# cnosdb/cnosdb

Hardware: NVIDIA H100
Metric: decoded+aggregated points/s (higher is better)
Workload: dtype i64/f64

## Files before the change

cnosdb_b200/csrc/scan_kernels.cuh:

```cuda
#pragma once
#include <type_traits>

#include "cursors.cuh"

namespace tskv {

constexpr uint32_t FULL = 0xffffffffu;
constexpr int MAX_RANGES = 8;
constexpr int N_TK = 3;
constexpr int N_VK = 3;
constexpr int N_SERIAL_BINS = N_TK * N_VK;
constexpr uint32_t SHORT_PAGE_ROWS = 1024;
enum { BIN_SHORT_RLE_S8B = N_SERIAL_BINS, BIN_SHORT_S8B_S8B = N_SERIAL_BINS + 1, BIN_SHORT_RLE_GOR = N_SERIAL_BINS + 2,
       BIN_SHORT_S8B_GOR = N_SERIAL_BINS + 3 };
constexpr int N_BINS = N_SERIAL_BINS + 4;

enum { TK_RLE = 0, TK_S8B = 1, TK_GEN = 2 };
enum { VK_S8B = 0, VK_GOR = 1, VK_GEN = 2 };

__host__ __device__ inline int time_class(uint8_t dk) {
  return dk == DK_RLE_SC ? TK_RLE : dk == DK_S8B_SC ? TK_S8B : TK_GEN;
}
__host__ __device__ inline int value_class(uint8_t dk) {
  return dk == DK_S8B_ZZ ? VK_S8B : dk == DK_GORILLA ? VK_GOR : VK_GEN;
// ... 656 lines not shown
  if (P.width <= 0) {
    b.lo = INT64_MIN; b.hi = INT64_MAX; b.idx = 0; b.valid = true; b.floor_regime = false;
    return true;
  }
  const int64_t w = P.width;
  const int64_t cap = P.floor_cap;
  if (b.valid && b.floor_regime && t > b.hi && (uint64_t)t - (uint64_t)b.hi <= (uint64_t)w && t <= cap &&
      b.idx + 1 < P.n_buckets) {
    b.lo = b.hi + 1;
    b.hi = (int64_t)((uint64_t)b.hi + ((uint64_t)cap - (uint64_t)b.hi < (uint64_t)w ? (uint64_t)cap - (uint64_t)b.hi : (uint64_t)w));
    b.idx += 1;
    return true;
  }
  int64_t dividend = (int64_t)((uint64_t)t - (uint64_t)P.origin_mod + (uint64_t)w);
  int64_t rem = dividend % w;
  int64_t start = (int64_t)((uint64_t)t - (uint64_t)rem);
  int64_t diff = (int64_t)((uint64_t)start - (uint64_t)P.first_bucket_start);
  if (diff < 0 || diff % w != 0 || diff / w >= (int64_t)P.n_buckets) return false;
  b.idx = (uint32_t)(diff / w);
  const bool wrapped = t < P.wrap_lo;
  if (dividend >= 0) {
    const uint64_t room = (uint64_t)(wrapped ? P.wrap_lo - 1 : cap) - (uint64_t)start;
    b.lo = start;
    b.hi = (int64_t)((uint64_t)start + (room < (uint64_t)(w - 1) ? room : (uint64_t)(w - 1)));
  } else {
    b.lo = start - w + 1; b.hi = start;
    if (b.lo < P.wrap_lo) b.lo = P.wrap_lo;
  }
  b.floor_regime = dividend >= 0 && !wrapped;
  b.valid = true;
  return true;
}

__device__ __forceinline__ bool range_span(const ScanParams &P, int64_t t, int64_t &lo, int64_t &hi) {
  lo = INT64_MIN;
  hi = INT64_MAX;
  if (P.n_ranges == 0) return true;
  if (P.n_ranges == 1) {
    const int64_t a = P.ranges[0].min_ts, b = P.ranges[0].max_ts;
    if (t < a) { hi = a - 1; return false; }
    if (t > b) { lo = b + 1; return false; }
    lo = a; hi = b;
    return true;
  }
  bool in = false;
#pragma unroll 1
  for (uint32_t k = 0; k < P.n_ranges; k++) {
    const int64_t a = P.ranges[k].min_ts, b = P.ranges[k].max_ts;
    if (t >= a && t <= b) {
      if (!in) { lo = a; hi = b; in = true; }
    } else if (!in) {
      if (a > t && a - 1 < hi) hi = a - 1;
      if (b < t && a <= b && b + 1 > lo) lo = b + 1;
    }
  }
  return in;
}

__device__ __forceinline__ bool tomb_span(const tskv_time_range *r, uint32_t n, int64_t t, int64_t &lo, int64_t &hi) {
  bool in = false;
  int64_t l = INT64_MIN, h = INT64_MAX;
#pragma unroll 1
  for (uint32_t k = 0; k < n; k++) {
    const int64_t a = r[k].min_ts, b = r[k].max_ts;
    if (a > b) continue;
    if (t >= a && t <= b) {
      if (!in) { l = a; h = b; in = true; }
    } else if (!in) {
      if (a > t && a - 1 < h) h = a - 1;
      if (b < t && b + 1 > l) l = b + 1;
    }
  }
  lo = lo > l ? lo : l;
  hi = hi < h ? hi : h;
  return in;
}

__device__ __forceinline__ uint4 tomb_lookup(const ScanParams &P, uint32_t series, uint32_t column) {
  uint4 out = make_uint4(0, 0, 0, 0);
#pragma unroll 1
  for (int pass = 0; pass < 2; pass++) {
    const uint64_t key = ((uint64_t)series << 32) | (pass == 0 ? (uint64_t)TSKV_TOMB_ALL : (uint64_t)column);
    uint32_t lo = 0, hi = P.n_tomb_keys;
    while (lo < hi) {
      const uint32_t mid = (lo + hi) >> 1;
      if (__ldg(P.tomb_keys + mid) < key) lo = mid + 1;
      else hi = mid;
    }
    if (lo < P.n_tomb_keys && __ldg(P.tomb_keys + lo) == key) {
      const uint32_t a = __ldg(P.tomb_off + lo), b = __ldg(P.tomb_off + lo + 1);
      if (pass == 0) { out.x = a; out.y = b - a; }
      else { out.z = a; out.w = b - a; }
    }
  }
  return out;
}

template <int VK>
struct ValueAcc {
  uint32_t count;
  uint64_t sum;
  int64_t sum_hi;
  int64_t kmin, kmax;
  __device__ __forceinline__ void reset(bool narrow = false) {
    count = 0; sum = 0; sum_hi = 0;
    kmin = narrow ? INT32_MAX : INT64_MAX;
    kmax = narrow ? INT32_MIN : INT64_MIN;
  }
  __device__ __forceinline__ static int64_t with_lo(int64_t x, int32_t lo) {
    return (int64_t)(((uint64_t)x & 0xffffffff00000000ull) | (uint32_t)lo);
  }
  __device__ __forceinline__ void add32(uint32_t v) {
    sum += (uint64_t)(int64_t)(int32_t)v;
    kmin = with_lo(kmin, min((int32_t)kmin, (int32_t)v));
    kmax = with_lo(kmax, max((int32_t)kmax, (int32_t)v));
  }
  __device__ __forceinline__ void add(uint64_t v, uint8_t pt, uint64_t flip, bool  = false) {
    int64_t key;
    if (VK == VK_GOR || (VK == VK_GEN && pt == TSKV_PT_F64)) {
      sum = (uint64_t)__double_as_longlong(__longlong_as_double((long long)sum) + __longlong_as_double((long long)v));
      key = (int64_t)(v ^ (uint64_t)(((int64_t)v >> 63) & 0x7fffffffffffffffll));
    } else {
      sum += (uint32_t)v;
      sum_hi += pt == TSKV_PT_I64 ? (int64_t)(int32_t)(v >> 32) : (int64_t)(v >> 32);
      key = (int64_t)(v ^ flip);
    }
    kmin = key < kmin ? key : kmin;
    kmax = key > kmax ? key : kmax;
  }
  __device__ __forceinline__ void fold(uint8_t pt, bool narrow = false) {
    if (VK == VK_GOR || (VK == VK_GEN && pt == TSKV_PT_F64)) return;
    if (narrow) {
      const uint64_t flip = pt == TSKV_PT_U64 ? 0x8000000000000000ull : 0ull;
      sum_hi = (int64_t)sum >> 63;
      kmin = (int64_t)((uint64_t)(int64_t)(int32_t)kmin ^ flip);
      kmax = (int64_t)((uint64_t)(int64_t)(int32_t)kmax ^ flip);
      return;
    }
    const uint64_t x = (uint64_t)sum_hi << 32;
    const uint64_t lo = x + sum;
    sum_hi = (pt == TSKV_PT_I64 ? (sum_hi >> 32) : (int64_t)((uint64_t)sum_hi >> 32)) + (lo < x ? 1 : 0);
    sum = lo;
  }
};

#ifdef TSKV_FLUSH_SLOTS
constexpr int FLUSH_SLOTS = TSKV_FLUSH_SLOTS;
__host__ __device__ constexpr int flush_slots(int ) { return FLUSH_SLOTS; }
#else
constexpr int FLUSH_SLOTS = 4;
__host__ __device__ constexpr int flush_slots(int tk) { return tk == TK_S8B ? 2 : FLUSH_SLOTS; }
#endif
constexpr int FLUSH_Q = 5;
__host__ __device__ constexpr uint32_t flush_stage_bytes(int ns) { return (ns * FLUSH_Q * 32 + ns) * 8; }

template <int VK, int NS>
__device__ __forceinline__ void reduce_staged(const ScanParams &P, uint64_t *stab, uint64_t *stage, uint32_t n_slots) {
  __syncwarp();
  const uint32_t lane = threadIdx.x & 31;
  const uint32_t s = lane & (NS - 1), g = lane / NS;
  const uint64_t meta = stage[NS * FLUSH_Q * 32 + s];
  const uint32_t qcol = (uint32_t)(meta >> 32);
  const ColState &cs = P.cols[s < n_slots ? qcol : 0];
  const bool is_f64 = VK == VK_GOR || (VK == VK_GEN && cs.phys_type == TSKV_PT_F64);
  uint64_t cnt = 0, sum = 0;
  int64_t hi = 0, kmin = INT64_MAX, kmax = INT64_MIN;
  const uint64_t *base = stage + (size_t)s * FLUSH_Q * 32;
  static_assert(NS == 2 || NS == 4, "reduce_staged: lane j owns slot j % NS");
#pragma unroll
  for (int i = 0; i < NS; i++) {
    const uint32_t src = g * NS + ((i + s) & (NS - 1));
    const uint64_t c = base[src], v = base[32 + src];
    cnt += c;
    if (is_f64) {
      sum = (uint64_t)__double_as_longlong(__longlong_as_double((long long)sum) + __longlong_as_double((long long)v));
    } else {
      sum += v;
      if (VK != VK_GOR) hi += (int64_t)base[64 + src] + (sum < v ? 1 : 0);
    }
    const int64_t a = (int64_t)base[96 + src], b = (int64_t)base[128 + src];
    kmin = a < kmin ? a : kmin;
    kmax = b > kmax ? b : kmax;
  }
#pragma unroll
  for (int o = NS; o < 32; o <<= 1) {
    cnt += shfl_xor_u64(cnt, o);
    const uint64_t v = shfl_xor_u64(sum, o);
    const int64_t vh = VK != VK_GOR ? (int64_t)shfl_xor_u64((uint64_t)hi, o) : 0;
    if (is_f64) {
      sum = (uint64_t)__double_as_longlong(__longlong_as_double((long long)sum) + __longlong_as_double((long long)v));
    } else {
      sum += v;
      if (VK != VK_GOR) hi += vh + (sum < v ? 1 : 0);
    }
    const int64_t a = (int64_t)shfl_xor_u64((uint64_t)kmin, o), b = (int64_t)shfl_xor_u64((uint64_t)kmax, o);
    kmin = a < kmin ? a : kmin;
    kmax = b > kmax ? b : kmax;
  }
  if (lane < n_slots && cnt)
    table_update(P, stab, cs, (uint64_t)(uint32_t)meta, cs.agg_mask, is_f64, (uint32_t)cnt, sum, hi, kmin, kmax);
  __syncwarp();
}

template <int VK, int NS>
__device__ __forceinline__ void stage_partial(const ScanParams &P, uint64_t *stab, uint64_t *stage, uint32_t &seq, bool live,
                                              const ValueAcc<VK> &va, bool meta_lane, uint64_t gcell) {
  uint64_t *q = stage + (size_t)seq * FLUSH_Q * 32 + (threadIdx.x & 31);
  q[0] = live ? va.count : 0;
  q[32] = live ? va.sum : 0;
  if (VK != VK_GOR) q[64] = live ? (uint64_t)va.sum_hi : 0;
  q[96] = live ? (uint64_t)va.kmin : (uint64_t)INT64_MAX;
  q[128] = live ? (uint64_t)va.kmax : (uint64_t)INT64_MIN;
  if (meta_lane) stage[NS * FLUSH_Q * 32 + seq] = gcell;
  if (++seq == NS) {
    reduce_staged<VK, NS>(P, stab, stage, seq);
    seq = 0;
  }
}

template <int VK, int NS>
__device__ __forceinline__ void flush_runs(const ScanParams &P, uint64_t *stab, uint64_t *stage, uint32_t &seq, bool active,
                                           uint32_t qcol, uint64_t cell, uint8_t pt, uint8_t mask, const ValueAcc<VK> &va) {
  const uint32_t m = __ballot_sync(FULL, active);
  if (m == 0) return;
  const uint32_t lane = threadIdx.x & 31;
  const uint64_t gcell = ((uint64_t)qcol << 32) | (uint32_t)cell;
  const int leader = __ffs(m) - 1;
  const uint64_t lcell = shfl_u64(gcell, leader);
  const bool same = !P.group_by_series && __all_sync(FULL, !active || gcell == lcell);
  if (same) {
    stage_partial<VK, NS>(P, stab, stage, seq, active && va.count, va, (int)lane == leader, lcell);
  } else if (active && va.count) {
    table_update(P, stab, P.cols[qcol], cell, mask, VK == VK_GOR || (VK == VK_GEN && pt == TSKV_PT_F64), va.count, va.sum,
                 va.sum_hi, va.kmin, va.kmax);
  }
}

template <int K, typename S>
__device__ __forceinline__ bool cursor_exhausted(const DeltaCursor<K, S> &c) { return c.exhausted; }
template <bool ZZ>
__device__ __forceinline__ bool cursor_exhausted(const S8bCursor<ZZ> &c) { return c.exhausted(); }
template <int K, typename S>
__device__ __forceinline__ void cursor_reset(DeltaCursor<K, S> &c, uint32_t lane_ring) { c.bs.reset(lane_ring); }
template <bool ZZ>
__device__ __forceinline__ void cursor_reset(S8bCursor<ZZ> &c, uint32_t lane_ring) { c.reset(lane_ring); }

__device__ __forceinline__ uint32_t rle_rows_within(uint64_t d, uint64_t delta, double inv, uint32_t left) {
  const double e = (double)d * inv;
  if (e >= (double)left) return left;
  uint64_t q = (uint64_t)e;
  if (__umul64hi(q, delta) != 0 || q * delta > d) q--;
  else if (d - q * delta >= delta) q++;
  return (uint32_t)min((uint64_t)left, q + 1);
}

__device__ __forceinline__ uint32_t edge_rows(const ScanParams &P, uint32_t b, uint64_t t, uint64_t delta, double inv) {
  if (b >= P.n_buckets) return 1u;
  const int64_t end = __ldg(P.edges + b + 1);
  return (int64_t)t < end ? rle_rows_within((uint64_t)end - 1 - t, delta, inv, 0xffffffffu) : 0u;
}

struct GenTimeCursor : DeltaCursor<-1, BeStream> {
  const uint32_t *bm = nullptr;
  uint32_t word = 0;
  bool none = false;
};

template <int TK, int VK, bool SEL, bool NARROW, bool EDGES>
__device__ __forceinline__ void scan_chunk_seg(const ScanParams &P, uint32_t item_begin, uint32_t item_end,
                                               uint32_t ring_base, uint64_t *stab, uint64_t *stage, uint4 *s_tomb,
                                               uint32_t part, uint32_t n_parts, uint32_t part_rows) {
  constexpr int NS = flush_slots(TK);
  const uint32_t lane = threadIdx.x & 31;
  const uint32_t item = item_begin + lane;
  const bool have_item = item < item_end;
  const uint32_t tslot = ring_base + lane * RING_BYTES;
  const uint32_t vslot = ring_base + (TK == TK_S8B ? RING_BYTES_PER_WARP : 0) + lane * RING_BYTES;

  uint32_t page = 0, slot = 0, qcol = 0, n_rows = 0;
  uint8_t pt = VK == VK_GOR ? TSKV_PT_F64 : TSKV_PT_I64, mask = 0;
  PageView tpv, vpv;
  typename std::conditional<TK == TK_GEN, GenTimeCursor, S8bCursor<false>>::type tcur;
  uint64_t rle_t0 = 0, rle_delta = 0;
  double rle_inv = 0.0;
  typename std::conditional<VK == VK_S8B, S8bCursor<true>, DeltaCursor<-1, SeqStream>>::type vcur_d;
  GorillaRing vcur_g;
  const uint32_t *vbm = nullptr;
  const uint32_t *keepw = nullptr;
  bool allnull = false;
  int64_t pend_t = 0;

  if constexpr (TK == TK_S8B) tcur.reset(tslot);
  if (VK == VK_GOR) vcur_g.reset(vslot);
  else cursor_reset(vcur_d, vslot);
  uint32_t r0 = 0, page_rows = 0;
  if (have_item) {
    page = P.work_page[item];
    slot = P.work_slot[item];
    qcol = P.work_qcol[item] & 0x7f;
    const tskv_page_desc vd = P.descs[page];
    if (P.has_tomb) s_tomb[threadIdx.x] = tomb_lookup(P, vd.series_id, vd.column_id);
    const uint32_t tpage = P.time_page_of[page];
    const tskv_page_desc td = P.descs[tpage];
    if (VK != VK_GOR) pt = P.cols[qcol].phys_type;
    mask = P.cols[qcol].agg_mask;
    page_rows = vd.num_values;
    uint32_t sk_v = SKIP_NONE, sk_t = SKIP_NONE;
    bool split = false;
    if (n_parts > 1 && page_rows > part_rows) {
      sk_v = __ldg(P.skip_off + page);
      sk_t = TK == TK_S8B ? __ldg(P.skip_off + tpage) : 0u;
      split = sk_v != SKIP_NONE && sk_t != SKIP_NONE;
    }
    r0 = part * part_rows;
    tskv_status st = kind_status(vd.reserved);
    uint32_t st_page = page;
    if constexpr (TK == TK_GEN) {
      if (kind_status(td.reserved) != TSKV_OK) { st = kind_status(td.reserved); st_page = tpage; }
    }
    if (part != 0 && (!split || r0 >= page_rows)) {
    } else if (st != TSKV_OK) {
      report_error(P, st, st_page);
    } else {
      tpv.open(P.arena, td);
      vpv.open(P.arena, vd);
      n_rows = split ? min(page_rows, r0 + part_rows) : page_rows;
      vbm = reinterpret_cast<const uint32_t *>(vpv.bitset);
      if (P.row_keep) keepw = P.row_keep + P.keep_off[tpage];
      const uint32_t ent = r0 / SKIP_ROWS - 1;
      if (TK == TK_RLE) {
        DeltaCursor<DK_RLE_SC, BeStream> rc;
        st = rc.open(tpv, td.reserved);
        rle_delta = rc.delta;
        rle_t0 = rc.v + rc.delta;
        if ((int64_t)rle_delta > 0) rle_inv = 1.0 / (double)rle_delta;
      } else if (part == 0) {
        st = tcur.open(tpv, td.reserved, tslot);
      } else if constexpr (TK == TK_S8B) {
        tcur.restore(tpv, tslot, load_skip(P.skip + sk_t + ent));
      }
      if (st == TSKV_OK) {
        if (part == 0) {
          if (VK == VK_GOR) vcur_g.open(vpv, vslot);
          else { st = vcur_d.open(vpv, vd.reserved, vslot); allnull = vd.reserved == DK_ALLNULL; }
        } else {
          const SkipEntry e = load_skip(P.skip + sk_v + ent);
          if constexpr (VK == VK_GOR) vcur_g.restore(vpv, vslot, e);
          else if constexpr (VK == VK_S8B) vcur_d.restore(vpv, vslot, e);
        }
      }
      if constexpr (TK == TK_GEN) {
        if (td.reserved == DK_ALLNULL) n_rows = 0;
        tcur.bm = reinterpret_cast<const uint32_t *>(tpv.bitset);
      }
      if (st == TSKV_OK && n_rows) {
        if (TK == TK_RLE) {
          pend_t = (int64_t)(rle_t0 + (uint64_t)r0 * rle_delta);
        } else if constexpr (TK == TK_GEN) {
          uint32_t f = 0, w = 0;
          while (f < n_rows && (w = __ldg(tcur.bm + (f >> 5))) == 0) f += 32;
          if (f < n_rows) f += __ffs(w) - 1;
          tcur.none = f >= n_rows;
          if (f == 0) {
            pend_t = (int64_t)tcur.next();
          } else if (!tcur.none) {
            tcur.skip_first_if_s8b_sc();
            DeltaCursor<-1, BeStream> peek = tcur;
            pend_t = (int64_t)peek.next();
          }
          tcur.word = __ldg(tcur.bm);
        } else if (part == 0) {
          pend_t = (int64_t)tcur.next();
        } else {
          pend_t = (int64_t)tcur.v;
        }
      }
      if (st != TSKV_OK) { report_error(P, st, st == TSKV_ERR_BITSET_MISMATCH ? tpage : page); n_rows = 0; }
    }
  }
  const bool to_page_end = n_rows == page_rows;
  ring_drain();

  static_assert(!NARROW || (VK == VK_S8B && !SEL), "narrow chunks: simple8b integer values, no FIRST / LAST");
  ValueAcc<VK> va;
  va.reset(NARROW);
  RunAcc acc;
  acc.first_ts = acc.last_ts = 0; acc.first_val = acc.last_val = 0; acc.first_ok = acc.last_ok = false;
  BucketState bk; bk.valid = false; bk.floor_regime = false; bk.lo = 0; bk.hi = 0; bk.idx = 0;
  bool have_run = false;
  uint32_t run_idx = 0;
  uint32_t row = r0;
  if (n_rows == 0) row = 0;
  uint32_t n_points = 0, n_inrange = 0;
  uint32_t vword = 0, vahead = vbm ? __ldg(vbm + (row >> 5)) : 0;
  uint32_t kword = 0xffffffffu;
  bool first_pending = false;
  const uint64_t flip = pt == TSKV_PT_U64 ? 0x8000000000000000ull : 0ull;
  const uint64_t group_base = SEL ? 0 : group_cell_base<EDGES>(P, slot);
  uint32_t staged = 0;

  auto flush_now = [&](bool flush) {
    if (flush) va.fold(pt, NARROW);
    if (SEL) {
      if (__any_sync(FULL, flush)) {
        acc.count = va.count; acc.sum = va.sum; acc.sum_hi = va.sum_hi; acc.kmin = va.kmin; acc.kmax = va.kmax;
        const uint32_t fslot = have_item ? __ldg(P.work_slot + item) : 0u;
        warp_flush<SEL, EDGES>(P, stab, flush, qcol, group_cell_base<EDGES>(P, fslot) + bucket_cell<EDGES>(P, run_idx, flush),
                               (int64_t)run_idx, pt, mask, acc, fslot);
      }
    } else {
      flush_runs<VK, NS>(P, stab, stage, staged, flush, qcol, group_base + bucket_cell<EDGES>(P, run_idx, flush), pt, mask, va);
    }
  };
  auto row_value = [&](bool accumulate, bool &vv, bool &kept) -> uint64_t {
    if ((row & 31) == 0) {
      vword = vahead;
      vahead = __ldg(vbm + (row >> 5) + 1);
      if constexpr (TK == TK_GEN) kword = (keepw ? __ldg(keepw + (row >> 5)) : 0xffffffffu) & tcur.word;
      else if (keepw) kword = __ldg(keepw + (row >> 5));
    }
    vv = ((vword >> (row & 31)) & 1) && !allnull;
    kept = (kword >> (row & 31)) & 1;
    uint64_t v = 0;
    if (vv) {
      n_points++;
      if constexpr (NARROW) {
        const uint32_t v32 = vcur_d.next32();
        if (accumulate && kept) { va.count++; va.add32(v32); }
      } else {
        v = VK == VK_GOR ? vcur_g.next() : vcur_d.next();
        if (accumulate && kept) { va.count++; va.add(v, pt, flip); }
      }
    }
    return v;
  };
  auto next_add = [&](bool take) {
    if constexpr (NARROW) {
      const uint32_t v32 = vcur_d.next32();
      if (take) va.add32(v32);
    } else {
      const uint64_t v = VK == VK_GOR ? vcur_g.next() : vcur_d.next();
      if (take) va.add(v, pt, flip);
    }
  };
  auto check_values = [&]() {
    const bool bad = VK == VK_GOR ? vcur_g.failed() : cursor_exhausted(vcur_d);
    if (bad) {
      report_error(P, (VK == VK_GOR && vcur_g.overran()) ? TSKV_ERR_SHORT_BLOCK : TSKV_ERR_BITSET_MISMATCH, page);
      n_rows = 0;
      have_run = false;
    }
  };

  uint32_t ra = 0, rb1 = 0, nb = 0xffffffffu, q32 = 0, bidx = 0;
  uint64_t e_off = 0, w_rem = 0;
  bool fast = false;
  if (TK == TK_RLE) {
    bool elig = P.n_ranges <= 1 && !P.has_tomb;
    if (elig && n_rows) {
      const uint64_t span_t = (uint64_t)(page_rows - 1) * rle_delta;
      elig = (int64_t)rle_delta > 0 && __umul64hi((uint64_t)(page_rows - 1), rle_delta) == 0 && span_t < (1ull << 62) &&
             rle_t0 + (1ull << 62) < (1ull << 63) && rle_t0 + span_t + (1ull << 62) < (1ull << 63) &&
             P.width < ((int64_t)1 << 61);
      if (elig) {
        const int64_t t0 = (int64_t)rle_t0;
        ra = 0;
        rb1 = page_rows;
        if (P.n_ranges == 1) {
          const int64_t a = P.ranges[0].min_ts, b = P.ranges[0].max_ts;
          ra = a <= t0 ? 0u : rle_rows_within((uint64_t)(a - 1) - rle_t0, rle_delta, rle_inv, page_rows);
          rb1 = b < t0 ? 0u : rle_rows_within((uint64_t)b - rle_t0, rle_delta, rle_inv, page_rows);
        }
        ra = min(max(ra, row), n_rows);
        rb1 = min(max(rb1, row), n_rows);
        if ((P.width > 0 || EDGES) && ra < rb1) {
          const int64_t tr = (int64_t)(rle_t0 + (uint64_t)ra * rle_delta);
          if (P.width > 0 && (int64_t)((uint64_t)tr - (uint64_t)P.origin_mod + (uint64_t)P.width) < 0) {
            elig = false;
          } else if (!locate_bucket<EDGES>(P, tr, bk)) {
            report_error(P, TSKV_ERR_BUCKET_RANGE, page);
            n_rows = 0;
          } else {
            bidx = bk.idx;
            nb = rle_rows_within((uint64_t)bk.hi - (uint64_t)tr, rle_delta, rle_inv, 0xffffffffu);
            if (P.width > 0) {
              e_off = (uint64_t)tr + (uint64_t)nb * rle_delta - ((uint64_t)bk.hi + 1);
              q32 = rle_rows_within((uint64_t)P.width, rle_delta, rle_inv, 0xffffffffu) - 1;
              w_rem = (uint64_t)P.width - (uint64_t)q32 * rle_delta;
            }
          }
        }
      }
    }
    fast = __all_sync(FULL, elig);
  }

  if (TK == TK_RLE && VK != VK_GEN && !SEL && fast && (P.width > 0 || EDGES) && !P.group_by_series) {
    const bool mine = row < n_rows;
    const uint32_t with_rows = __ballot_sync(FULL, mine);
    const int src = with_rows ? __ffs(with_rows) - 1 : 0;
    const uint64_t t_first = rle_t0 + (uint64_t)row * rle_delta;
    const bool agree = (shfl_u64(rle_delta, src) == rle_delta) & (shfl_u64(t_first, src) == t_first) &
                       (shfl_u64(e_off, src) == e_off) & (__shfl_sync(FULL, row, src) == row) &
                       (__shfl_sync(FULL, n_rows, src) == n_rows) & (__shfl_sync(FULL, ra, src) == ra) &
                       (__shfl_sync(FULL, rb1, src) == rb1) & (__shfl_sync(FULL, bidx, src) == bidx) &
                       (__shfl_sync(FULL, nb, src) == nb) & (__shfl_sync(FULL, qcol, src) == qcol) &
                       (__shfl_sync(FULL, (uint32_t)group_base, src) == (uint32_t)group_base);
    if (with_rows && __all_sync(FULL, !mine || agree)) {
      rle_delta = shfl_u64(rle_delta, src);
      e_off = shfl_u64(e_off, src);
      w_rem = shfl_u64(w_rem, src);
      q32 = __shfl_sync(FULL, q32, src);
      row = __shfl_sync(FULL, row, src);
      ra = __shfl_sync(FULL, ra, src);
      rb1 = __shfl_sync(FULL, rb1, src);
      bidx = __shfl_sync(FULL, bidx, src);
      nb = __shfl_sync(FULL, nb, src);
      if (EDGES) {
        rle_t0 = shfl_u64(rle_t0, src);
        rle_inv = __longlong_as_double((long long)shfl_u64((uint64_t)__double_as_longlong(rle_inv), src));
      }
      const uint64_t col = ((uint64_t)__shfl_sync(FULL, qcol, src) << 32) | __shfl_sync(FULL, (uint32_t)group_base, src);
      uint32_t end = __shfl_sync(FULL, n_rows, src);
      while (row < end) {
        if (n_rows) {
          vword = vahead;
          vahead = __ldg(vbm + (row >> 5) + 1);
          if (keepw) kword = __ldg(keepw + (row >> 5));
        }
        const uint32_t wend = min(row + 32, end);
        const uint32_t m = (n_rows && !allnull) ? vword & (0xffffffffu >> (32 - (wend - row))) : 0u;
        const uint32_t lo = min(max(ra, row), wend) - row, hi = max(min(max(rb1, row), wend) - row, lo);
        const uint32_t take = m & kword & (uint32_t)((1ull << hi) - (1ull << lo));
        const bool dense = __all_sync(FULL, take == m);
        uint32_t r = row;
        while (r < wend) {
          const bool in = r >= ra && r < rb1;
          uint32_t pend = r < ra ? min(ra, wend) : wend;
          if (in) {
            if (nb == 0) {
              if (EDGES) {
                do {
                  bidx++;
                  nb = edge_rows(P, bidx, rle_t0 + (uint64_t)r * rle_delta, rle_delta, rle_inv);
                } while (nb == 0);
              } else {
                do {
                  bidx++;
                  nb = q32 + (e_off < w_rem ? 1u : 0u);
                  e_off = e_off + (uint64_t)nb * rle_delta - (uint64_t)P.width;
                } while (nb == 0);
              }
// ... 58 lines not shown
            } else {
              nb = q32 + (e_off < w_rem ? 1u : 0u);
              e_off = e_off + (uint64_t)nb * rle_delta - (uint64_t)P.width;
            }
          }
          if (bidx >= P.n_buckets) {
            report_error(P, TSKV_ERR_BUCKET_RANGE, page);
            seg_in = false;
            n_rows = row;
            pending = false;
          } else {
            seg_n = min(nb, rb1 - row);
            seg_b = bidx;
            if (P.width > 0 || EDGES) nb -= seg_n;
          }
        }
      } else {
        lim_lo = lim_hi = pend_t;
        seg_in = range_span(P, pend_t, lim_lo, lim_hi);
        if constexpr (TK == TK_GEN) seg_in = seg_in && !tcur.none;
        if (P.has_tomb) {
          const uint4 tl = s_tomb[threadIdx.x];
          const bool dropped = tomb_span(P.tomb_ranges, P.n_tomb_global, pend_t, lim_lo, lim_hi) |
                               tomb_span(P.tomb_ranges + tl.x, tl.y, pend_t, lim_lo, lim_hi);
          seg_masked = tomb_span(P.tomb_ranges + tl.z, tl.w, pend_t, lim_lo, lim_hi);
          if (dropped) seg_in = false;
        }
        if (seg_in) {
          if (!(bk.valid && pend_t >= bk.lo && pend_t <= bk.hi) && !locate_bucket<EDGES>(P, pend_t, bk)) {
            report_error(P, TSKV_ERR_BUCKET_RANGE, page);
            seg_in = false;
            bk.valid = false;
            lim_lo = lim_hi = pend_t;
          } else {
            lim_lo = lim_lo > bk.lo ? lim_lo : bk.lo;
            lim_hi = lim_hi < bk.hi ? lim_hi : bk.hi;
            seg_b = bk.idx;
          }
        }
        if (TK == TK_RLE) {
          const uint32_t left = n_rows - row;
          if ((int64_t)rle_delta > 0) {
            seg_n = rle_rows_within((uint64_t)lim_hi - (uint64_t)pend_t, rle_delta, rle_inv, left);
          } else {
            int64_t t = pend_t;
            do {
              seg_n++;
              t = (int64_t)((uint64_t)t + rle_delta);
            } while (seg_n < left && t >= lim_lo && t <= lim_hi);
          }
        }
      }
    }
    bool go = pending;
    if (align) {
      const uint32_t bmin = __reduce_min_sync(FULL, (pending && seg_in) ? seg_b : 0xffffffffu);
      go = pending && (!seg_in || seg_b == bmin);
    }
    const bool newrun = go && seg_in && (!have_run || seg_b != run_idx);
    const bool flush = have_run && (newrun || !has);
    flush_now(flush);
    if (flush) have_run = false;
    if (newrun) {
      have_run = true;
      run_idx = seg_b;
      va.reset(NARROW);
      if (SEL) { acc.first_ok = acc.last_ok = false; first_pending = true; }
    }
    if (go) {
      pending = false;
      const bool accumulate = seg_in && !seg_masked;
      if (TK == TK_RLE) {
        const uint32_t rend = row + seg_n;
        uint32_t r = row;
        while (r < rend) {
          if ((r & 31) == 0) {
            vword = vahead;
            vahead = __ldg(vbm + (r >> 5) + 1);
            if (keepw) kword = __ldg(keepw + (r >> 5));
          }
          const uint32_t off = r & 31;
          const uint32_t span = min(32u - off, rend - r);
          const uint32_t smask = 0xffffffffu >> (32 - span);
          const uint32_t m = allnull ? 0u : ((vword >> off) & smask);
          const uint32_t kb = (kword >> off) & smask;
          n_points += __popc(m);
          if (seg_in) n_inrange += __popc(kb);
          if (!SEL) {
            const uint32_t take = accumulate ? (m & kb) : 0u;
            va.count += __popc(take);
            if (__all_sync(__activemask(), take == m)) {
#pragma unroll 1
              for (uint32_t n = __popc(m); n; n--) next_add(true);
            } else {
#pragma unroll 1
              for (uint32_t b = m; b; b &= b - 1) next_add(take & b & (0u - b));
            }
          } else {
            for (uint32_t j = 0; j < span; j++) {
              bool vv = (m >> j) & 1;
              uint64_t v = 0;
              if (vv) v = VK == VK_GOR ? vcur_g.next() : vcur_d.next();
              vv = vv && !seg_masked;
              if (seg_in && ((kb >> j) & 1)) {
                const int64_t t = (int64_t)(rle_t0 + (uint64_t)(r + j) * rle_delta);
                if (first_pending) { acc.first_ts = t; acc.first_val = vv ? v : 0; acc.first_ok = vv; first_pending = false; }
                acc.last_ts = t;
                acc.last_val = vv ? v : 0;
                acc.last_ok = vv;
                if (vv) { va.count++; va.add(v, pt, flip); }
              }
            }
          }
          r += span;
        }
        row = rend;
        if (!(TK == TK_RLE && fast)) pend_t = (int64_t)(rle_t0 + (uint64_t)rend * rle_delta);
      } else {
        int64_t t = pend_t;
        const uint64_t span = (uint64_t)lim_hi - (uint64_t)lim_lo;
        bool more;
#pragma unroll 1
        do {
          bool vv, kept;
          const uint64_t v = row_value(accumulate, vv, kept);
          if (SEL && seg_in && kept) {
            const bool ok = vv && !seg_masked;
            if (first_pending) { acc.first_ts = t; acc.first_val = ok ? v : 0; acc.first_ok = ok; first_pending = false; }
            acc.last_ts = t;
            acc.last_val = ok ? v : 0;
            acc.last_ok = ok;
          }
          if (seg_in && kept) n_inrange++;
          row++;
          if constexpr (TK == TK_GEN) {
            if (row < n_rows) {
              if ((row & 31) == 0) tcur.word = __ldg(tcur.bm + (row >> 5));
              if ((tcur.word >> (row & 31)) & 1) t = (int64_t)tcur.next();
            }
          } else {
            t = (int64_t)tcur.next();
          }
          more = row < n_rows && (uint64_t)t - (uint64_t)lim_lo <= span;
        } while (more);
        pend_t = t;
        if (cursor_exhausted(tcur) && (TK == TK_GEN || row < n_rows)) {
          report_error(P, TSKV_ERR_BITSET_MISMATCH, P.time_page_of[page]);
          n_rows = row;
        }
      }
      check_values();
    }
  }
  if (!SEL && staged) {
    reduce_staged<VK, NS>(P, stab, stage, staged);
    staged = 0;
  }
  if (VK == VK_GOR && have_item && n_rows != 0 && to_page_end && vcur_g.consumed_any() && !vcur_g.drain())
    report_error(P, TSKV_ERR_SHORT_BLOCK, page);
  ring_drain();
  n_points = __reduce_add_sync(FULL, n_points);
  n_inrange = __reduce_add_sync(FULL, n_inrange);
  if (lane == 0) {
    if (n_points) atomicAdd(&P.stats[0], (unsigned long long)n_points);
    if (n_inrange) atomicAdd(&P.stats[1], (unsigned long long)n_inrange);
  }
}

#ifndef SCAN_MIN_BLOCKS
#define SCAN_MIN_BLOCKS 4
#endif
__host__ __device__ constexpr int scan_min_blocks(int , bool ) { return SCAN_MIN_BLOCKS; }
__host__ __device__ constexpr uint32_t scan_ring_bytes_per_warp(int tk) {
  return tk == TK_S8B ? 2 * RING_BYTES_PER_WARP : RING_BYTES_PER_WARP;
}
__host__ __device__ constexpr uint32_t scan_warp_bytes(int tk) {
  return scan_ring_bytes_per_warp(tk) + flush_stage_bytes(flush_slots(tk));
}
constexpr uint32_t SCAN_TOMB_BYTES = SCAN_THREADS * sizeof(uint4);
enum { NARROW_NONE = 0, NARROW_SOME = 1, NARROW_ALL = 2 };
template <int TK, int VK, bool SEL, int NARROW, bool EDGES>
__global__ void __launch_bounds__(SCAN_THREADS, scan_min_blocks(TK, SEL)) k_scan_aggregate(const __grid_constant__ ScanParams P, int bin) {
  static_assert(NARROW == NARROW_NONE || (TK != TK_GEN && VK == VK_S8B && !SEL), "narrow kernels: simple8b values, no FIRST / LAST");
  extern __shared__ __align__(16) uint64_t s_tab[];
  if (P.use_smem) {
    for (uint32_t i = threadIdx.x; i < P.smem_words; i += SCAN_THREADS) s_tab[i] = 0;
    __syncthreads();
    for (uint32_t c = 0; c < P.n_cols; c++) {
      const ColState cs = P.cols[c];
      for (uint32_t i = threadIdx.x; i < (uint32_t)P.n_cells; i += SCAN_THREADS) {
        if (cs.agg_mask & TSKV_AGG_MIN) s_tab[cs.s_min + i] = 0x7fffffffffffffffull;
        if (cs.agg_mask & TSKV_AGG_MAX) s_tab[cs.s_max + i] = 0x8000000000000000ull;
      }
    }
    __syncthreads();
  }
  const uint32_t lane = threadIdx.x & 31;
  uint64_t *warp_area = s_tab + ((P.smem_words + 1) & ~1u) + (size_t)(threadIdx.x >> 5) * (scan_warp_bytes(TK) / 8);
  const uint32_t ring_base = (uint32_t)__cvta_generic_to_shared(warp_area);
  uint64_t *stage = warp_area + scan_ring_bytes_per_warp(TK) / 8;
  uint4 *s_tomb = reinterpret_cast<uint4 *>(s_tab + ((P.smem_words + 1) & ~1u) + (SCAN_THREADS / 32) * (scan_warp_bytes(TK) / 8));
  uint32_t n_groups = 0;
  for (uint32_t k = bin * P.n_cols * WL_SUB; k < (bin + 1) * P.n_cols * WL_SUB; k++) n_groups += (__ldg(P.region_fill + k) + 31) >> 5;
  const uint32_t n_parts = (TK == TK_GEN || VK == VK_GEN || SEL) ? 1u : P.bin_parts[bin];
  const uint32_t part_rows = P.bin_part_rows[bin];
  const uint32_t n_chunks = n_groups * n_parts;
  for (;;) {
    uint32_t c = 0;
    if (lane == 0) c = atomicAdd(P.task_counter + bin, 1u);
    c = __shfl_sync(FULL, c, 0);
    if (c >= n_chunks) break;
    uint32_t group = n_parts > 1 ? c / n_parts : c;
    const uint32_t part = c - group * n_parts;
    uint32_t k = bin * P.n_cols * WL_SUB;
    asm("" : "+r"(k));
    uint32_t fill = __ldg(P.region_fill + k);
    while (group >= (fill + 31) >> 5) {
      group -= (fill + 31) >> 5;
      fill = __ldg(P.region_fill + ++k);
    }
    const uint32_t region = __ldg(P.region_start + k);
    const uint32_t begin = region + (group << 5);
    const uint32_t end = min(begin + 32, region + fill);
    if constexpr (NARROW == NARROW_SOME) {
      const uint32_t item = begin + lane;
      const bool narrow = __all_sync(FULL, item >= end || __ldg(P.page_narrow + __ldg(P.work_page + item)));
      if (narrow) scan_chunk_seg<TK, VK, SEL, true, EDGES>(P, begin, end, ring_base, s_tab, stage, s_tomb, part, n_parts, part_rows);
      else scan_chunk_seg<TK, VK, SEL, false, EDGES>(P, begin, end, ring_base, s_tab, stage, s_tomb, part, n_parts, part_rows);
    } else {
      scan_chunk_seg<TK, VK, SEL, NARROW == NARROW_ALL, EDGES>(P, begin, end, ring_base, s_tab, stage, s_tomb, part, n_parts, part_rows);
    }
  }
  if (P.use_smem) {
    __syncthreads();
    for (uint32_t c = 0; c < P.n_cols; c++) {
      const ColState cs = P.cols[c];
      const bool f64 = cs.phys_type == TSKV_PT_F64;
      for (uint32_t i = threadIdx.x; i < (uint32_t)P.n_cells; i += SCAN_THREADS) {
        const uint64_t cnt = s_tab[cs.s_count + i];
        if (!cnt) continue;
        atomicAdd(reinterpret_cast<unsigned long long *>(P.state + cs.count_off + i), (unsigned long long)cnt);
        if (cs.agg_mask & (TSKV_AGG_SUM | TSKV_AGG_MEAN)) {
          const uint64_t sv = s_tab[cs.s_sum + i];
          if (f64) atomicAdd(reinterpret_cast<double *>(P.state + cs.sum_off + i), __longlong_as_double((long long)sv));
          else add_int_sum(P.state + cs.sum_off + i, P.state + cs.sumhi_off + i, cs.agg_mask, sv,
                           (cs.agg_mask & TSKV_AGG_MEAN) ? (int64_t)s_tab[cs.s_hi + i] : 0);
        }
        if (cs.agg_mask & TSKV_AGG_MIN) atomicMin(reinterpret_cast<long long *>(P.state + cs.min_off + i), (long long)s_tab[cs.s_min + i]);
        if (cs.agg_mask & TSKV_AGG_MAX) atomicMax(reinterpret_cast<long long *>(P.state + cs.max_off + i), (long long)s_tab[cs.s_max + i]);
      }
    }
  }
}

struct StateLayout {
  uint64_t sum_i64_off, sum_i64_len;
  uint64_t sum_f64_off, sum_f64_len;
  uint64_t min_off, min_len;
  uint64_t max_off, max_len;
  uint64_t selval_off, selval_len;
  uint64_t first_pairs_off, first_cells;
  uint64_t last_pairs_off, last_cells;
  uint64_t first_keys_off, last_keys_off;
  uint64_t snap_off;
  uint64_t total;
};

constexpr uint32_t AUX_TASK_COUNTERS = 0;
constexpr uint32_t AUX_STATUS = 8;
constexpr uint32_t AUX_ERR_PAGE = 9;
constexpr uint32_t AUX_STATS = 10;
constexpr uint32_t AUX_COUNTERS = 12;
constexpr uint32_t AUX_CRC_STATUS = AUX_COUNTERS + N_COUNTERS;
constexpr uint32_t AUX_CRC_ERR_PAGE = AUX_CRC_STATUS + 1;
constexpr uint32_t AUX_WORDS = 32;
static_assert(N_BINS * 4 <= (AUX_STATUS - AUX_TASK_COUNTERS) * 8 && AUX_CRC_ERR_PAGE < AUX_WORDS, "scan aux block layout");

__global__ void k_init_state(uint64_t *state, StateLayout L, unsigned long long *aux, uint32_t aux_words, uint32_t *zero32,
                             uint32_t n_zero32) {
  uint64_t i = (uint64_t)blockIdx.x * blockDim.x + threadIdx.x;
  uint64_t stride = (uint64_t)gridDim.x * blockDim.x;
  for (uint64_t k = i; k < aux_words; k += stride) aux[k] = 0;
  for (uint64_t k = i; k < n_zero32; k += stride) zero32[k] = 0;
  for (uint64_t k = i; k < L.total; k += stride) {
    uint64_t v = 0;
    if (k >= L.min_off && k < L.min_off + L.min_len) v = 0x7fffffffffffffffull;
    else if (k >= L.max_off && k < L.max_off + L.max_len) v = 0x8000000000000000ull;
    else if (k >= L.first_pairs_off && k < L.first_pairs_off + 2 * L.first_cells) v = ((k - L.first_pairs_off) & 1) ? 0 : 0x7fffffffffffffffull;
    else if (k >= L.last_pairs_off && k < L.last_pairs_off + 2 * L.last_cells) v = ((k - L.last_pairs_off) & 1) ? 0 : 0x8000000000000000ull;
    state[k] = v;
  }
}

struct MeanExport {
  uint64_t lo_off, hi_off, dst_off;
  uint32_t is_signed, pad;
};

__global__ void k_export_pairs(uint64_t *state, StateLayout L, const MeanExport *means, uint32_t n_means,
                               uint64_t n_cells) {
  uint64_t i = (uint64_t)blockIdx.x * blockDim.x + threadIdx.x;
  uint64_t stride = (uint64_t)gridDim.x * blockDim.x;
  for (uint32_t m = 0; m < n_means; m++) {
    const MeanExport me = means[m];
    for (uint64_t k = i; k < n_cells; k += stride) {
      uint64_t lo = state[me.lo_off + k];
      int64_t hi = (int64_t)state[me.hi_off + k];
      double d;
      if (me.is_signed) d = (double)(((__int128)hi << 64) + (__int128)(unsigned __int128)lo);
      else d = (double)(((unsigned __int128)(uint64_t)hi << 64) | (unsigned __int128)lo);
      state[me.dst_off + k] = (uint64_t)__double_as_longlong(d);
    }
  }
  for (uint64_t k = i; k < L.first_cells; k += stride) {
    state[L.first_keys_off + k] = state[L.first_pairs_off + 2 * k];
    state[L.selval_off + k] = state[L.first_pairs_off + 2 * k + 1];
  }
  for (uint64_t k = i; k < L.last_cells; k += stride) {
    state[L.last_keys_off + k] = state[L.last_pairs_off + 2 * k];
    state[L.selval_off + L.first_cells + k] = state[L.last_pairs_off + 2 * k + 1];
  }
}

enum { COMBINE_ADD = 0, COMBINE_INT_SUM = 1, COMBINE_F64_SUM = 2, COMBINE_MIN = 3, COMBINE_MAX = 4 };
struct CombineOp {
  uint64_t pane_off, win_off;
  uint64_t pane_hi_off, win_hi_off;
  uint32_t kind, has_hi;
};

__global__ void k_window_combine(const uint64_t *pane, uint64_t *win, const CombineOp *ops, uint32_t n_groups,
                                 uint32_t n_windows, uint32_t n_panes, uint32_t k) {
  const CombineOp op = ops[blockIdx.y];
  const uint64_t n = (uint64_t)n_groups * n_windows;
  for (uint64_t c = (uint64_t)blockIdx.x * blockDim.x + threadIdx.x; c < n; c += (uint64_t)gridDim.x * blockDim.x) {
    const uint64_t g = c / n_windows;
    const uint32_t j = (uint32_t)(c - g * n_windows);
    const uint32_t p0 = j + 1 >= k ? j + 1 - k : 0, p1 = j < n_panes - 1 ? j : n_panes - 1;
    const uint64_t *src = pane + op.pane_off + g * n_panes;
    switch (op.kind) {
      case COMBINE_INT_SUM: {
        const uint64_t *src_hi = pane + op.pane_hi_off + g * n_panes;
        uint64_t lo = 0, hi = 0;
        for (uint32_t p = p0; p <= p1; p++) {
          const uint64_t v = src[p];
          lo += v;
          hi += (lo < v ? 1u : 0u) + (op.has_hi ? src_hi[p] : 0u);
        }
        win[op.win_off + c] = lo;
        if (op.has_hi) win[op.win_hi_off + c] = hi;
        break;
      }
      case COMBINE_F64_SUM: {
        double acc = 0.0;
        for (uint32_t p = p0; p <= p1; p++) acc += __longlong_as_double((long long)src[p]);
        win[op.win_off + c] = (uint64_t)__double_as_longlong(acc);
        break;
      }
      case COMBINE_MIN: {
        int64_t acc = INT64_MAX;
        for (uint32_t p = p0; p <= p1; p++) acc = (int64_t)src[p] < acc ? (int64_t)src[p] : acc;
        win[op.win_off + c] = (uint64_t)acc;
        break;
      }
      case COMBINE_MAX: {
        int64_t acc = INT64_MIN;
        for (uint32_t p = p0; p <= p1; p++) acc = (int64_t)src[p] > acc ? (int64_t)src[p] : acc;
        win[op.win_off + c] = (uint64_t)acc;
        break;
      }
      default: {
        uint64_t acc = 0;
        for (uint32_t p = p0; p <= p1; p++) acc += src[p];
        win[op.win_off + c] = acc;
      }
    }
  }
}

__global__ void k_snapshot_keys(uint64_t *state, StateLayout L) {
  uint64_t i = (uint64_t)blockIdx.x * blockDim.x + threadIdx.x;
  uint64_t stride = (uint64_t)gridDim.x * blockDim.x;
  for (uint64_t k = i; k < L.first_cells; k += stride) state[L.snap_off + k] = state[L.first_keys_off + k];
  for (uint64_t k = i; k < L.last_cells; k += stride) state[L.snap_off + L.first_cells + k] = state[L.last_keys_off + k];
}
// ... 137 lines not shown
```

Baseline: 135.7 billion.

## Batch reduced flush partials into a per-warp ring before table updates

For the four-slot flush path, reduced partials are written into a 32-entry shared-memory ring instead of each being applied to the aggregation table immediately. When the ring fills, or at kernel end, all 32 lanes apply their updates in parallel. This replaces many narrow table updates done by at most four lanes with fewer full-warp updates, and the ring now persists across chunks. The cost is extra shared memory per warp (which may reduce occupancy) and more complex tail and drain bookkeeping.

```diff
diff --git a/cnosdb_b200/csrc/scan_kernels.cuh b/cnosdb_b200/csrc/scan_kernels.cuh
--- a/cnosdb_b200/csrc/scan_kernels.cuh
+++ b/cnosdb_b200/csrc/scan_kernels.cuh
@@ -832,10 +832,32 @@
 __host__ __device__ constexpr int flush_slots(int tk) { return tk == TK_S8B ? 2 : FLUSH_SLOTS; }
 #endif
 constexpr int FLUSH_Q = 5;
-__host__ __device__ constexpr uint32_t flush_stage_bytes(int ns) { return (ns * FLUSH_Q * 32 + ns) * 8; }
+constexpr uint32_t FLUSH_RING = 32;
+__host__ __device__ constexpr bool flush_ring(int ns) { return ns == 4; }
+__host__ __device__ constexpr uint32_t flush_stage_bytes(int ns) {
+  return (ns * FLUSH_Q * 32 + ns) * 8 + (flush_ring(ns) ? FLUSH_RING * (FLUSH_Q + 1) * 8 : 0);
+}
+template <int NS>
+__device__ __forceinline__ uint64_t *ring_of(uint64_t *stage) { return stage + NS * FLUSH_Q * 32 + NS; }
+
+template <int VK>
+__device__ __forceinline__ void drain_ring(const ScanParams &P, uint64_t *stab, const uint64_t *ring, uint32_t n) {
+  __syncwarp();
+  const uint32_t lane = threadIdx.x & 31;
+  const uint64_t cnt = lane < n ? ring[lane] : 0;
+  if (cnt) {
+    const uint64_t meta = ring[FLUSH_Q * FLUSH_RING + lane];
+    const ColState &cs = P.cols[(uint32_t)(meta >> 32)];
+    const bool is_f64 = VK == VK_GOR || (VK == VK_GEN && cs.phys_type == TSKV_PT_F64);
+    table_update(P, stab, cs, (uint64_t)(uint32_t)meta, cs.agg_mask, is_f64, (uint32_t)cnt, ring[FLUSH_RING + lane],
+                 (int64_t)ring[2 * FLUSH_RING + lane], (int64_t)ring[3 * FLUSH_RING + lane], (int64_t)ring[4 * FLUSH_RING + lane]);
+  }
+  __syncwarp();
+}
 
 template <int VK, int NS>
-__device__ __forceinline__ void reduce_staged(const ScanParams &P, uint64_t *stab, uint64_t *stage, uint32_t n_slots) {
+__device__ __forceinline__ void reduce_staged(const ScanParams &P, uint64_t *stab, uint64_t *stage, uint32_t n_slots,
+                                              uint32_t rpos) {
   __syncwarp();
   const uint32_t lane = threadIdx.x & 31;
   const uint32_t s = lane & (NS - 1), g = lane / NS;
@@ -877,24 +899,66 @@
     kmin = a < kmin ? a : kmin;
     kmax = b > kmax ? b : kmax;
   }
-  if (lane < n_slots && cnt)
+  if constexpr (flush_ring(NS)) {
+    if (lane < NS) {
+      uint64_t *e = ring_of<NS>(stage) + rpos + lane;
+      e[0] = lane < n_slots ? cnt : 0;
+      e[FLUSH_RING] = sum;
+      e[2 * FLUSH_RING] = (uint64_t)hi;
+      e[3 * FLUSH_RING] = (uint64_t)kmin;
+      e[4 * FLUSH_RING] = (uint64_t)kmax;
+      e[FLUSH_Q * FLUSH_RING] = meta;
+    }
+  } else if (lane < n_slots && cnt) {
     table_update(P, stab, cs, (uint64_t)(uint32_t)meta, cs.agg_mask, is_f64, (uint32_t)cnt, sum, hi, kmin, kmax);
+  }
   __syncwarp();
+}
+
+template <int VK, int NS>
+__device__ __forceinline__ void flush_staged_tail(const ScanParams &P, uint64_t *stab, uint64_t *stage, uint32_t &seq) {
+  if constexpr (!flush_ring(NS)) {
+    if (seq) reduce_staged<VK, NS>(P, stab, stage, seq, 0);
+    seq = 0;
+    return;
+  }
+  const uint32_t part = seq & (NS - 1);
+  if (!part) return;
+  const uint32_t rpos = seq - part;
+  reduce_staged<VK, NS>(P, stab, stage, part, rpos);
+  seq = rpos + NS;
+  if (seq == FLUSH_RING) {
+    drain_ring<VK>(P, stab, ring_of<NS>(stage), FLUSH_RING);
+    seq = 0;
+  }
 }
 
 template <int VK, int NS>
 __device__ __forceinline__ void stage_partial(const ScanParams &P, uint64_t *stab, uint64_t *stage, uint32_t &seq, bool live,
                                               const ValueAcc<VK> &va, bool meta_lane, uint64_t gcell) {
-  uint64_t *q = stage + (size_t)seq * FLUSH_Q * 32 + (threadIdx.x & 31);
+  const uint32_t slot = flush_ring(NS) ? seq & (NS - 1) : seq;
+  uint64_t *q = stage + (size_t)slot * FLUSH_Q * 32 + (threadIdx.x & 31);
   q[0] = live ? va.count : 0;
   q[32] = live ? va.sum : 0;
   if (VK != VK_GOR) q[64] = live ? (uint64_t)va.sum_hi : 0;
   q[96] = live ? (uint64_t)va.kmin : (uint64_t)INT64_MAX;
   q[128] = live ? (uint64_t)va.kmax : (uint64_t)INT64_MIN;
-  if (meta_lane) stage[NS * FLUSH_Q * 32 + seq] = gcell;
-  if (++seq == NS) {
-    reduce_staged<VK, NS>(P, stab, stage, seq);
-    seq = 0;
+  if (meta_lane) stage[NS * FLUSH_Q * 32 + slot] = gcell;
+  if constexpr (!flush_ring(NS)) {
+    if (++seq == NS) {
+      reduce_staged<VK, NS>(P, stab, stage, seq, 0);
+      seq = 0;
+    }
+  } else if (slot == NS - 1) {
+    reduce_staged<VK, NS>(P, stab, stage, NS, seq + 1 - NS);
+    if (seq + 1 == FLUSH_RING) {
+      drain_ring<VK>(P, stab, ring_of<NS>(stage), FLUSH_RING);
+      seq = 0;
+    } else {
+      seq++;
+    }
+  } else {
+    seq++;
   }
 }
 
@@ -948,8 +1012,8 @@
 
 template <int TK, int VK, bool SEL, bool NARROW, bool EDGES>
 __device__ __forceinline__ void scan_chunk_seg(const ScanParams &P, uint32_t item_begin, uint32_t item_end,
-                                               uint32_t ring_base, uint64_t *stab, uint64_t *stage, uint4 *s_tomb,
-                                               uint32_t part, uint32_t n_parts, uint32_t part_rows) {
+                                               uint32_t ring_base, uint64_t *stab, uint64_t *stage, uint32_t &staged,
+                                               uint4 *s_tomb, uint32_t part, uint32_t n_parts, uint32_t part_rows) {
   constexpr int NS = flush_slots(TK);
   const uint32_t lane = threadIdx.x & 31;
   const uint32_t item = item_begin + lane;
@@ -1077,7 +1141,6 @@
   bool first_pending = false;
   const uint64_t flip = pt == TSKV_PT_U64 ? 0x8000000000000000ull : 0ull;
   const uint64_t group_base = SEL ? 0 : group_cell_base<EDGES>(P, slot);
-  uint32_t staged = 0;
 
   auto flush_now = [&](bool flush) {
     if (flush) va.fold(pt, NARROW);
@@ -1442,10 +1505,7 @@
       check_values();
     }
   }
-  if (!SEL && staged) {
-    reduce_staged<VK, NS>(P, stab, stage, staged);
-    staged = 0;
-  }
+  if (!SEL) flush_staged_tail<VK, NS>(P, stab, stage, staged);
   if (VK == VK_GOR && have_item && n_rows != 0 && to_page_end && vcur_g.consumed_any() && !vcur_g.drain())
     report_error(P, TSKV_ERR_SHORT_BLOCK, page);
   ring_drain();
@@ -1495,6 +1555,7 @@
   const uint32_t n_parts = (TK == TK_GEN || VK == VK_GEN || SEL) ? 1u : P.bin_parts[bin];
   const uint32_t part_rows = P.bin_part_rows[bin];
   const uint32_t n_chunks = n_groups * n_parts;
+  uint32_t staged = 0;
   for (;;) {
     uint32_t c = 0;
     if (lane == 0) c = atomicAdd(P.task_counter + bin, 1u);
@@ -1512,15 +1573,17 @@
     const uint32_t region = __ldg(P.region_start + k);
     const uint32_t begin = region + (group << 5);
     const uint32_t end = min(begin + 32, region + fill);
+    if constexpr (!flush_ring(flush_slots(TK))) staged = 0;
     if constexpr (NARROW == NARROW_SOME) {
       const uint32_t item = begin + lane;
       const bool narrow = __all_sync(FULL, item >= end || __ldg(P.page_narrow + __ldg(P.work_page + item)));
-      if (narrow) scan_chunk_seg<TK, VK, SEL, true, EDGES>(P, begin, end, ring_base, s_tab, stage, s_tomb, part, n_parts, part_rows);
-      else scan_chunk_seg<TK, VK, SEL, false, EDGES>(P, begin, end, ring_base, s_tab, stage, s_tomb, part, n_parts, part_rows);
+      if (narrow) scan_chunk_seg<TK, VK, SEL, true, EDGES>(P, begin, end, ring_base, s_tab, stage, staged, s_tomb, part, n_parts, part_rows);
+      else scan_chunk_seg<TK, VK, SEL, false, EDGES>(P, begin, end, ring_base, s_tab, stage, staged, s_tomb, part, n_parts, part_rows);
     } else {
-      scan_chunk_seg<TK, VK, SEL, NARROW == NARROW_ALL, EDGES>(P, begin, end, ring_base, s_tab, stage, s_tomb, part, n_parts, part_rows);
-    }
-  }
+      scan_chunk_seg<TK, VK, SEL, NARROW == NARROW_ALL, EDGES>(P, begin, end, ring_base, s_tab, stage, staged, s_tomb, part, n_parts, part_rows);
+    }
+  }
+  if (!SEL && flush_ring(flush_slots(TK)) && staged) drain_ring<VK>(P, s_tab, ring_of<flush_slots(TK)>(stage), staged);
   if (P.use_smem) {
     __syncthreads();
     for (uint32_t c = 0; c < P.n_cols; c++) {
```

Result: faster. 139.5 billion (median of 6 runs) (+2.8%).
